# Jamol/kuma

Hardware: AMD Instinct MI355X
Metric: GiB/s device-resident WS frame mask/unmask, 64 KiB frames; % HBM peak (higher is better)
Workload: dtype u8

## Files before the change

### kuma_amd/csrc/kmws_utf8.hip

```cpp
#include "kmws_common.hpp"
#include "kmws_unmask_tile.hpp"
#include "kmws_utf8_dev.hpp"
#include "kmws_utf8_rule.hpp"

namespace kmws {

constexpr uint32_t kStatusBadStreams = kStatusBadDesc;

struct Utf8Ws {
    size_t plan_bytes;
    size_t first_bad, elems, aggs, pre, carry, total;
    uint32_t nblk;
};
static Utf8Ws utf8_ws_behind(size_t plan_bytes, uint32_t n, uint32_t n_streams)
{
    Utf8Ws w;
    w.nblk = (n + kBlock - 1) / kBlock;
    w.plan_bytes = plan_bytes;
    w.first_bad = r16(w.plan_bytes);
    w.elems = w.first_bad + r16((size_t)n * 4);
    w.aggs = w.elems + r16((size_t)n * 8);
    w.pre = w.aggs + r16((size_t)w.nblk * 8);
    w.carry = w.pre + r16((size_t)w.nblk * 8);
    w.total = w.carry + r16((size_t)n_streams * 8);
    return w;
}
static Utf8Ws utf8_ws(uint64_t span, uint32_t n, uint32_t n_streams)
{
    return utf8_ws_behind(kmws_unmask_workspace_size(span), n, n_streams);
}

__device__ __forceinline__ Utf8Elem block_scan(Utf8Elem e, Utf8Elem* s)
{
    const int tid = threadIdx.x;
    s[tid] = e;
    __syncthreads();
#pragma unroll
    for (int dlt = 1; dlt < kBlock; dlt <<= 1) {
        const Utf8Elem t = tid >= dlt ? utf8_combine(s[tid - dlt], s[tid]) : s[tid];
        __syncthreads();
        s[tid] = t;
        __syncthreads();
    }
    return s[tid];
}

__device__ __forceinline__ uint32_t stream_of(const uint32_t* __restrict__ first, uint32_t ns, uint32_t i)
{
    if (!first) return 0u;
    uint32_t lo = 0, hi = ns - 1;
    while (lo < hi) {
        const uint32_t mid = lo + (hi - lo + 1) / 2;
        if (first[mid] <= i) lo = mid; else hi = mid - 1;
    }
    return lo;
}
__device__ __forceinline__ uint32_t stream_begin(const uint32_t* __restrict__ first, uint32_t s)
{
    return first ? first[s] : 0u;
}
__device__ __forceinline__ uint32_t stream_end(const uint32_t* __restrict__ first, uint32_t n, uint32_t s)
{
    return first ? first[s + 1] : n;
}

__device__ __forceinline__ uint64_t load_carry(const kmws_utf8_carry* __restrict__ c, uint32_t s)
{
    uint64_t x = 0;
    if (c)
        for (int k = 0; k < 8; ++k) x |= (uint64_t)c[s].b[k] << (8 * k);
    return x;
}
__device__ __forceinline__ void store_carry(kmws_utf8_carry* __restrict__ c, uint32_t s, uint64_t x)
{
    for (int k = 0; k < 8; ++k) c[s].b[k] = (uint8_t)(x >> (8 * k));
}

__global__ void __launch_bounds__(kBlock) utf8_elem_kernel(const uint8_t* __restrict__ base, uint64_t span,
                                                           const kmws_desc* __restrict__ d,
                                                           const uint16_t* __restrict__ flags, uint32_t n, int masked,
                                                           const uint32_t* __restrict__ first, uint32_t ns,
                                                           const kmws_utf8_carry* __restrict__ carry_in,
                                                           Utf8Elem* __restrict__ elems, uint32_t* __restrict__ first_bad,
                                                           Utf8Elem* __restrict__ aggs, uint32_t nblk,
                                                           WsHead* __restrict__ head)
{
    __shared__ Utf8Elem s_scan[kBlock];
    const uint32_t i = blockIdx.x * kBlock + threadIdx.x;
    if (first && i <= ns) {
        const uint32_t x = first[i];
        if ((i == 0 && x != 0u) || (i == ns && x != n) || (i < ns && x > first[i + 1]))
            atomicOr(&head->status, kStatusBadStreams);
    }
    Utf8Elem e = utf8_identity();
    if (i < n) {
        const kmws_desc df = d[i];
        const uint32_t ob = flags[i] & 0xFFu, op = ob & 0x0Fu;
        uint32_t nb = 0, tail = 0;
        if (df.off > span || df.off + (uint64_t)df.len > span) {
            atomicOr(&head->status, kStatusBadDesc);
        } else if (op < 8u) {
            nb = df.len < 3u ? df.len : 3u;
            for (uint32_t k = 0; k < nb; ++k) {
                const uint32_t j = df.len - nb + k;
                uint32_t b = base[df.off + j];
                if (masked) b ^= (df.key >> (8u * (j & 3u))) & 0xFFu;
                tail = (tail << 8) | b;
            }
        }
        e = utf8_frame_elem(ob, i, tail, nb);
        uint32_t fb = kUtf8None;
        const uint32_t s = stream_of(first, ns, i);
        if (stream_begin(first, s) == i) {
            bool bad = false;
            const Utf8Elem st = utf8_carry_unpack(load_carry(carry_in, s), i, &bad);
            e = utf8_combine(st, e);
            if (bad && (op == 0u || op >= 8u)) fb = 0u;
        }
        elems[i] = e;
        first_bad[i] = fb;
    }
    const Utf8Elem inc = block_scan(e, s_scan);
    if (threadIdx.x == kBlock - 1 && blockIdx.x < nblk) aggs[blockIdx.x] = inc;
}

__global__ void __launch_bounds__(kBlock) utf8_scan_aggs_kernel(const Utf8Elem* __restrict__ aggs,
                                                                Utf8Elem* __restrict__ pre, uint32_t nblk)
{
    __shared__ Utf8Elem s_scan[kBlock];
    Utf8Elem run = utf8_identity();
    for (uint32_t c0 = 0; c0 < nblk; c0 += kBlock) {
        const uint32_t b = c0 + threadIdx.x;
        const Utf8Elem e = b < nblk ? aggs[b] : utf8_identity();
        block_scan(e, s_scan);
        const Utf8Elem ex = threadIdx.x ? s_scan[threadIdx.x - 1] : utf8_identity();
        if (b < nblk) pre[b] = utf8_combine(run, ex);
        run = utf8_combine(run, s_scan[kBlock - 1]);
        __syncthreads();
    }
}

__global__ void __launch_bounds__(kBlock) utf8_ctx_kernel(const uint16_t* __restrict__ flags, uint32_t n,
                                                          const uint32_t* __restrict__ first, uint32_t ns,
                                                          const kmws_utf8_carry* __restrict__ carry_in,
                                                          Utf8Elem* __restrict__ elems, const Utf8Elem* __restrict__ pre,
                                                          uint32_t* __restrict__ first_bad,
                                                          Utf8Elem* __restrict__ carry_tmp)
{
    __shared__ Utf8Elem s_scan[kBlock];
    const uint32_t i = blockIdx.x * kBlock + threadIdx.x;
    const Utf8Elem e = i < n ? elems[i] : utf8_identity();
    block_scan(e, s_scan);
    if (i >= n) return;
    Utf8Elem before = utf8_combine(pre[blockIdx.x], threadIdx.x ? s_scan[threadIdx.x - 1] : utf8_identity());
    const Utf8Elem after = utf8_combine(before, e);
    const uint32_t s = stream_of(first, ns, i);
    if (stream_begin(first, s) == i) {
        bool bad = false;
        before = utf8_carry_unpack(load_carry(carry_in, s), i, &bad);
    }
    const uint32_t ob = flags[i] & 0xFFu;
    const Utf8View v = utf8_frame_view(before, ob, i);
    elems[i] = Utf8Elem{v.slot, v.w};
    if ((v.w & kUtf8Checked) && (ob & 0x80u)) {
        const uint32_t nb = utf8_elem_nb(e);
        const uint32_t L = nb >= 3u ? utf8_elem_ctx(e) : (((v.w << (8u * nb)) | utf8_elem_ctx(e)) & 0xFFFFFFu);
        if (utf8_pending(L)) atomicMin(&first_bad[v.slot], i + 1u);
    }
    if (i + 1u == stream_end(first, n, s)) carry_tmp[s] = after;
}

constexpr int kUtf8V = (int)(kPlanTile / 16 / kBlock);
constexpr int kUtf8PolLoad = 2;
constexpr int kUtf8RsrcWord3 = 0x00020000;

__device__ __forceinline__ void covered_tile_check(const u32x4 (&v)[kUtf8V], const uint32_t (&prev)[kUtf8V],
                                                   uint32_t r, uint64_t lo, const kmws_desc& d0, Utf8View fv,
                                                   uint32_t f, uint32_t* __restrict__ first_bad)
{
    const int tid = threadIdx.x, lane = tid & 63;
    const uint64_t end = d0.off + d0.len;
    bool slow[kUtf8V];
    bool any = false;
#pragma unroll
    for (int i = 0; i < kUtf8V; ++i) {
        const uint64_t a = lo + 16u * (uint64_t)(tid + kBlock * i);
        const u32x4 w = v[i] ^ r;
        const uint32_t hb = (w.x | w.y | w.z | w.w) & 0x80808080u;
        slow[i] = hb != 0u || ((prev[i] ^ r) & 0x80000000u) != 0u || a < d0.off + 3u;
        any |= slow[i];
    }
    bool bad = false;
    if (__any(any)) {
#pragma unroll
        for (int i = 0; i < kUtf8V; ++i) {
            const uint64_t a = lo + 16u * (uint64_t)(tid + kBlock * i);
            if (slow[i]) bad |= word_bad(prev[i] ^ r, v[i] ^ r, a, d0.off, end, fv.w);
        }
    }
    const unsigned long long m = __ballot(bad);
    if (m != 0ull && lane == __ffsll((long long)m) - 1) report_bad(first_bad, fv.slot, f);
}

template <bool MASKED>
__device__ __forceinline__ void frames_check(const u32x4 (&v)[kUtf8V], const uint32_t (&prev)[kUtf8V], uint64_t lo,
                                             uint64_t hi, const kmws_desc* __restrict__ d, uint32_t f, uint32_t fl,
                                             const Utf8View* __restrict__ views, uint32_t* __restrict__ first_bad)
{
    const int tid = threadIdx.x;
#pragma unroll
    for (int i = 0; i < kUtf8V; ++i) {
        const uint64_t a = lo + 16u * (uint64_t)(tid + kBlock * i);
        if (a >= hi) continue;
        uint32_t gl = f, gh = fl + 1u;
        while (gl < gh) {
            const uint32_t mid = gl + (gh - gl) / 2;
            const kmws_desc dm = d[mid];
            if (dm.off + dm.len <= a) gl = mid + 1; else gh = mid;
        }
        for (uint32_t g = gl; g <= fl; ++g) {
            const kmws_desc dg = d[g];
            if (dg.off >= a + 16u) break;
            if (dg.len == 0u) continue;
            const Utf8View gv = views[g];
            if (!(gv.w & kUtf8Checked)) continue;
            const uint32_t r = MASKED ? rot_key(dg.key, dg.off) : 0u;
            if (plain_word_frame_bad(v[i] ^ r, prev[i] ^ r, a, dg.off, dg.off + dg.len, gv.w))
                report_bad(first_bad, gv.slot, g);
        }
    }
}

template <bool MASKED>
__global__ void __launch_bounds__(kBlock, MASKED ? 4 : 7) utf8_payload_kernel(const uint8_t* __restrict__ base, uint64_t span,
                                                              const kmws_desc* __restrict__ d, uint32_t n,
                                                              const TileRec* __restrict__ map,
                                                              const WsHead* __restrict__ head,
                                                              const Utf8View* __restrict__ views,
                                                              uint32_t* __restrict__ first_bad, TileMapping tm,
                                                              uint32_t b0)
{
    const int tid = threadIdx.x, lane = tid & 63, wave = tid >> 6;
    const uint32_t tile = tile_of_block(b0 + blockIdx.x, tm);
    const uint64_t lo = (uint64_t)tile * kPlanTile;
    const uint64_t hi = lo + kPlanTile < span ? lo + kPlanTile : span;
    const TileRecPair recs = *reinterpret_cast<const TileRecPair*>(map + tile);
    if (head->status != 0u) return;
    const bool cov = tile_rec_covered(recs.at, n);
    const uint32_t f = tile_rec_frame(recs.at, n);
    uint32_t fl = tile_rec_frame(recs.next, n);
    if (f >= n) return;
    if (fl >= n) fl = n - 1;
    if (fl < f) fl = f;

    Utf8View fv = Utf8View{0u, 0u};
    kmws_desc d0 = kmws_desc{0ull, 0u, 0u};
    if (cov) {
        fv = views[f];
        if (!(fv.w & kUtf8Checked)) return;
        d0 = d[f];
    } else {
        bool any = false;
        for (uint32_t g = f + (uint32_t)tid; g <= fl; g += kBlock) any |= (views[g].w & kUtf8Checked) != 0u;
        if (!__syncthreads_or(any)) return;
    }

    const __amdgpu_buffer_rsrc_t rs = __builtin_amdgcn_make_buffer_rsrc(
        const_cast<uint8_t*>(base) + lo, (short)0, (int)((hi - lo + 15) & ~15ull), kUtf8RsrcWord3);
    u32x4 v[kUtf8V];
#pragma unroll
    for (int i = 0; i < kUtf8V; ++i) {
        const uint32_t x = 16u * (uint32_t)(tid + kBlock * i);
        if (lo + x < hi) v[i] = __builtin_amdgcn_raw_buffer_load_b128(rs, (int)x, 0, kUtf8PolLoad);
        else v[i] = u32x4{0, 0, 0, 0};
    }
    uint32_t edge = 0;
    if (lane < kUtf8V) {
        const uint64_t ae = lo + 16u * (uint64_t)(64 * wave + kBlock * lane);
        if (ae >= 4u && ae <= span) edge = *reinterpret_cast<const uint32_t*>(base + ae - 4);
    }
    uint32_t prev[kUtf8V];
#pragma unroll
    for (int i = 0; i < kUtf8V; ++i) {
        const uint32_t up = __shfl_up(v[i].w, 1);
        const uint32_t ed = __shfl(edge, i);
        prev[i] = lane == 0 ? ed : up;
    }

    if (cov) {
        covered_tile_check(v, prev, MASKED ? recs.at.rkey : 0u, lo, d0, fv, f, first_bad);
        return;
    }

    frames_check<MASKED>(v, prev, lo, hi, d, f, fl, views, first_bad);
}

__global__ void __launch_bounds__(kBlock) utf8_finish_kernel(uint32_t n, const uint32_t* __restrict__ first,
                                                             uint32_t ns, const Utf8View* __restrict__ views,
                                                             const uint32_t* __restrict__ first_bad,
                                                             const Utf8Elem* __restrict__ carry_tmp,
                                                             const kmws_utf8_carry* __restrict__ carry_in,
                                                             kmws_utf8_carry* __restrict__ carry_out,
                                                             uint8_t* __restrict__ out)
{
    const uint32_t i = blockIdx.x * kBlock + threadIdx.x;
    if (i < n) {
        const Utf8View v = views[i];
        uint8_t r = KMWS_UTF8_NOT_TEXT;
        if (v.w & kUtf8Checked) {
            const uint32_t fb = first_bad[v.slot];
            r = fb > i + 1u ? KMWS_UTF8_OK : (fb == i + 1u ? KMWS_UTF8_BAD : KMWS_UTF8_AFTER_BAD);
        }
        out[i] = r;
    }
    if (carry_out && i < ns) {
        const uint32_t s = i;
        uint64_t c;
        if (stream_begin(first, s) >= stream_end(first, n, s)) {
            c = load_carry(carry_in, s);
        } else {
            const Utf8Elem after = carry_tmp[s];
            const bool chk = (after.w & (kUtf8Open | kUtf8Checked)) == (kUtf8Open | kUtf8Checked);
            c = utf8_carry_pack(after, chk && after.slot < n && first_bad[after.slot] != kUtf8None);
        }
        store_carry(carry_out, s, c);
    }
}

__global__ void __launch_bounds__(kBlock) utf8_carry_copy_kernel(uint32_t ns,
                                                                 const kmws_utf8_carry* __restrict__ carry_in,
                                                                 kmws_utf8_carry* __restrict__ carry_out)
{
    const uint32_t s = blockIdx.x * kBlock + threadIdx.x;
    if (s < ns) store_carry(carry_out, s, load_carry(carry_in, s));
}

constexpr int kFusedRows = (int)(kPlanTile / 1024);
constexpr uint32_t kFusedNoStore = 0x7FFFFFF0u;
static_assert(kUtf8V == kUnmaskV && kFusedRows == 4 * kUtf8V, "the validator's tile is the apply's");

constexpr unsigned kFusedBlocksPerCu = 4;
constexpr unsigned kFusedStaticLds = kUnmaskStaticLds + 4u * (unsigned)kFusedRows;

struct FusedWs {
    Utf8Ws u;
    size_t edges, total;
};
static FusedWs fused_ws(uint64_t span, uint32_t n, uint32_t n_streams)
{
    FusedWs w;
    w.u = utf8_ws(span, n, n_streams);
    const uint64_t ntiles = (span + kPlanTile - 1) / kPlanTile;
    w.edges = r16(w.u.total);
    w.total = w.edges + r16((size_t)ntiles * 4);
    return w;
}

__global__ void __launch_bounds__(kBlock) utf8_edges_kernel(const uint8_t* __restrict__ base,
                                                            uint32_t* __restrict__ edges, uint32_t ntiles)
{
    const uint32_t t = blockIdx.x * kBlock + threadIdx.x;
    if (t < ntiles) edges[t] = t ? *reinterpret_cast<const uint32_t*>(base + (uint64_t)t * kPlanTile - 4) : 0u;
}

__device__ __forceinline__ void fused_lookback(const u32x4 (&v)[kUtf8V], uint32_t edge, uint32_t* s_row,
                                               uint32_t (&prev)[kUtf8V])
{
    const int lane = threadIdx.x & 63, wave = threadIdx.x >> 6;
    if (lane == 63) {
#pragma unroll
        for (int i = 0; i < kUtf8V; ++i) s_row[wave + 4 * i] = v[i].w;
    }
    __syncthreads();
#pragma unroll
    for (int i = 0; i < kUtf8V; ++i) {
        const uint32_t up = __shfl_up(v[i].w, 1);
        const uint32_t ed = (wave == 0 && i == 0) ? edge : s_row[wave + 4 * i - 1];
        prev[i] = lane == 0 ? ed : up;
    }
}

__device__ __forceinline__ bool fused_word_frame_bad(const u32x4& v, uint32_t prev, uint64_t a, uint64_t off,
                                                     uint64_t end, uint32_t r, uint32_t ctx)
{
    return plain_word_frame_bad(v ^ r, prev ^ r, a, off, end, ctx);
}

template <bool FULL, bool TWO, bool NT>
__device__ __forceinline__ void fused_tile(uint8_t* __restrict__ base, uint64_t tile_lo, uint64_t tile_hi,
                                           const kmws_desc* __restrict__ d, uint32_t n, TileRec rec, TileRec rec_next,
                                           bool ok, const u32x4 (&v)[kUtf8V], uint32_t edge,
                                           const Utf8View* __restrict__ views, uint32_t* __restrict__ first_bad,
                                           uint64_t* s_off, uint64_t* s_end, uint32_t* s_key, uint32_t* s_row,
                                           const u32x4* pre)
{
    constexpr int V = kUtf8V;
    using Cfg = UnmaskCfg<V>;
    constexpr int SP = !NT ? kPolPlain : (TWO ? kPolStreamStoreLarge : kPolStreamStoreSmall);
    const int tid = threadIdx.x;
    const __amdgpu_buffer_rsrc_t rs = tile_rsrc(base, tile_lo, tile_hi);

    if (FULL && tile_rec_covered(rec, n)) {
        const uint32_t r = rec.rkey;
        const uint32_t f = tile_rec_frame(rec, n);
        const uint32_t fi = f < n ? f : 0u;
        const Utf8View fv = views[fi];
        const kmws_desc d0 = d[fi];
        const __amdgpu_buffer_rsrc_t rs_ok = __builtin_amdgcn_make_buffer_rsrc(
            base + tile_lo, (short)0, ok ? (int)Cfg::kTile : 0, kBufferRsrcWord3);
#pragma unroll
        for (int i = 0; i < V; ++i) {
            __builtin_amdgcn_sched_barrier(0);
            store_word<SP>(v[i] ^ r, rs_ok, 16u * (uint32_t)(tid + kBlock * i));
        }
        __builtin_amdgcn_sched_barrier(0);
        if (!ok | (f >= n) | !(fv.w & kUtf8Checked) | (d0.len == 0u) | (d0.off > tile_lo)) return;
        uint32_t prev[V];
        fused_lookback(v, edge, s_row, prev);
        covered_tile_check(v, prev, r, tile_lo, d0, fv, f, first_bad);
        return;
    }

    const uint32_t f0 = tile_rec_frame(rec, n);
    const uint32_t flast = tile_rec_frame(rec_next, n);
    const kmws_desc d0 = d[f0 < n ? f0 : 0];

    if (TWO && FULL && flast <= f0 + 1 && f0 < n) {
        const bool two = flast > f0 && flast < n;
        const kmws_desc d1 = two ? d[flast] : kmws_desc{~0ull, 0u, 0u};
        u32x4 m[V];
        const auto [r0, r1, s0, t0, s1, t1] = two_frame_masks(tile_lo, d0, d1, tid, m);
        const Utf8View v0 = views[f0];
        const Utf8View v1 = two ? views[flast] : Utf8View{0u, 0u};
        __builtin_amdgcn_sched_barrier(0);
#pragma unroll
        for (int i = 0; i < V; ++i) {
            const bool st = ok && (m[i].x | m[i].y | m[i].z | m[i].w) != 0u;
            store_word<SP>(v[i] ^ m[i], rs, st ? 16u * (uint32_t)(tid + kBlock * i) : kFusedNoStore);
        }
        if (!ok) return;
        const bool c0 = (v0.w & kUtf8Checked) != 0u && t0 > s0, c1 = (v1.w & kUtf8Checked) != 0u && t1 > s1;
        if (!c0 && !c1) return;
        uint32_t prev[V];
        fused_lookback(v, edge, s_row, prev);
#pragma unroll
        for (int i = 0; i < V; ++i) {
            const uint32_t x = 16u * (uint32_t)(tid + kBlock * i);
            const uint64_t a = tile_lo + x;
            if (c0 && s0 < x + 16 && t0 > x &&
                fused_word_frame_bad(v[i], prev[i], a, d0.off, d0.off + d0.len, r0, v0.w))
                report_bad(first_bad, v0.slot, f0);
            if (c1 && s1 < x + 16 && t1 > x &&
                fused_word_frame_bad(v[i], prev[i], a, d1.off, d1.off + d1.len, r1, v1.w))
                report_bad(first_bad, v1.slot, flast);
        }
        return;
    }

    u32x4 m[V];
    staged_masks(tile_lo, tile_hi, d, n, f0, flast, pre, s_off, s_end, s_key, tid, m);
    bool any = false;
    uint32_t fl = flast >= n ? n - 1 : flast;
    if (fl < f0) fl = f0;
    if (ok && f0 < n)
        for (uint32_t g = f0 + (uint32_t)tid; g <= fl; g += kBlock) any |= (views[g].w & kUtf8Checked) != 0u;
    if (__syncthreads_or(any)) {
        uint32_t prev[V];
        fused_lookback(v, edge, s_row, prev);
        frames_check<true>(v, prev, tile_lo, tile_hi, d, f0, fl, views, first_bad);
    }
#pragma unroll
    for (int i = 0; i < V; ++i) {
        const uint32_t x = 16u * (uint32_t)(tid + kBlock * i);
        const u32x4 mm = m[i];
        const bool st = ok && (mm.x | mm.y | mm.z | mm.w) != 0u;
        store_word<SP>(v[i] ^ mm, rs, st ? x : kFusedNoStore);
    }
}

template <bool TWO, bool NT>
__global__ void __launch_bounds__(kBlock) unmask_utf8_split_kernel(uint8_t* __restrict__ base,
                                                                   const kmws_desc* __restrict__ d, uint32_t n,
                                                                   const TileRec* __restrict__ map,
                                                                   const WsHead* __restrict__ head,
                                                                   const Utf8View* __restrict__ views,
                                                                   uint32_t* __restrict__ first_bad,
                                                                   const uint32_t* __restrict__ edges, TileMapping tm,
                                                                   uint32_t b0)
{
    using Cfg = UnmaskCfg<kUtf8V>;
    __shared__ uint64_t s_off[Cfg::kCap];
    __shared__ uint64_t s_end[Cfg::kCap];
    __shared__ uint32_t s_key[Cfg::kCap];
    __shared__ uint32_t s_row[kFusedRows];
    const uint32_t tile = tile_of_block(b0 + blockIdx.x, tm);
    const uint64_t lo = (uint64_t)tile * Cfg::kTile;
    const TileRecPair recs = *reinterpret_cast<const TileRecPair*>(map + tile);
    const TileRec rec = recs.at, rec_next = recs.next;
    const uint32_t status = head->status;
    const uint32_t edge = edges[tile];
    u32x4 v[kUtf8V];
    if constexpr (!TWO) {
        const uint32_t f = tile_rec_frame(rec, n), fl = tile_rec_frame(rec_next, n);
        const uint32_t fi = f + threadIdx.x;
        u32x4 pre = u32x4{0, 0, 0, 0};
        if (fi < n && fi <= fl) pre = *reinterpret_cast<const u32x4*>(d + fi);
        load_tile<kUtf8V, true>(base, lo, lo + Cfg::kTile, v);
        __builtin_amdgcn_sched_barrier(0);
        fused_tile<true, TWO, NT>(base, lo, lo + Cfg::kTile, d, n, rec, rec_next, (status & kStatusBadDesc) == 0, v,
                                  edge, views, first_bad, s_off, s_end, s_key, s_row, &pre);
        return;
    }
    __builtin_amdgcn_sched_barrier(0);
    load_tile<kUtf8V, true>(base, lo, lo + Cfg::kTile, v);
    __builtin_amdgcn_sched_barrier(0);
    fused_tile<true, TWO, NT>(base, lo, lo + Cfg::kTile, d, n, rec, rec_next, (status & kStatusBadDesc) == 0, v, edge,
                              views, first_bad, s_off, s_end, s_key, s_row, nullptr);
}

__global__ void __launch_bounds__(kBlock) unmask_utf8_tail_kernel(uint8_t* __restrict__ base, uint64_t span,
                                                                  const kmws_desc* __restrict__ d, uint32_t n,
                                                                  const TileRec* __restrict__ map,
                                                                  const WsHead* __restrict__ head,
                                                                  const Utf8View* __restrict__ views,
                                                                  uint32_t* __restrict__ first_bad,
                                                                  const uint32_t* __restrict__ edges, uint32_t tile)
{
    using Cfg = UnmaskCfg<kUtf8V>;
    __shared__ uint64_t s_off[Cfg::kCap];
    __shared__ uint64_t s_end[Cfg::kCap];
    __shared__ uint32_t s_key[Cfg::kCap];
    __shared__ uint32_t s_row[kFusedRows];
    const uint64_t tile_lo = (uint64_t)tile * Cfg::kTile;
    const uint32_t edge = edges[tile];
    u32x4 v[kUtf8V];
    load_tile<kUtf8V, false>(base, tile_lo, span, v);
    __builtin_amdgcn_sched_barrier(0);
    fused_tile<false, false, true>(base, tile_lo, span, d, n, map[tile], map[tile + 1],
                                   (head->status & kStatusBadDesc) == 0, v, edge, views, first_bad, s_off, s_end,
                                   s_key, s_row, nullptr);
}

static_assert(kPieceWords == kUtf8V * kBlock, "a piece is a tile of the validator: fused_lookback's rows");
__global__ void __launch_bounds__(kBlock) unmask_pieces_utf8_kernel(uint8_t* __restrict__ base,
                                                                    const kmws_desc* __restrict__ d,
                                                                    const Utf8View* __restrict__ views,
                                                                    const PieceRecEdge* __restrict__ pieces,
                                                                    uint8_t* __restrict__ verdict)
{
    constexpr int V = kUtf8V;
    __shared__ uint32_t s_row[kFusedRows];
    const PieceRecEdge pr = pieces[blockIdx.x];
    const kmws_desc x = d[pr.frame];
    const Utf8View fv = views[pr.frame];
    const PieceHull h = piece_hull(x, pr.piece);
    u32x4 v[V];
    load_piece(base, h, v);
    if (x.key != 0u) store_piece(base, x, h, v);
    if (!(fv.w & kUtf8Checked)) return;
    uint32_t prev[V];
    fused_lookback(v, pr.piece ? pr.edge : 0u, s_row, prev);
    bool bad = false;
#pragma unroll
    for (int i = 0; i < V; ++i) {
        const uint64_t w = h.w0 + threadIdx.x + (uint64_t)kBlock * i;
        if (w < h.w1) bad |= fused_word_frame_bad(v[i], prev[i], 16 * w, x.off, h.end, h.r, fv.w);
    }
    const unsigned long long m = __ballot(bad);
    if (m != 0ull && (int)(threadIdx.x & 63) == __ffsll((long long)m) - 1) verdict[fv.slot] = (uint8_t)1;
}

kmws_status launch_unmask_pieces_utf8(uint8_t* base, const kmws_desc* descs, const Utf8View* views,
                                      const PieceRecEdge* pieces, uint32_t np, uint8_t* verdict, hipStream_t s)
{
    if (np == 0) return KMWS_OK;
    if (!base || !descs || !views || !pieces || !verdict) return KMWS_ERR_INVALID_PARAM;
    hipLaunchKernelGGL(unmask_pieces_utf8_kernel, dim3(np), dim3(kBlock), 0, s, base, descs, views, pieces, verdict);
    return hip_status(hipGetLastError());
}

static bool have_device()
{
    static const bool have = kmws_device_count() > 0;
    return have;
}

kmws_status utf8_stream_args_check(bool ptrs_ok, const void* a, const void* b, uint32_t n, const uint32_t* stream_first,
                                   uint32_t n_streams, size_t need, size_t have)
{
    if (n >= 0x80000000u || n_streams >= 0x80000000u) return KMWS_ERR_INVALID_PARAM;
    if (n && !ptrs_ok) return KMWS_ERR_INVALID_PARAM;
    if ((reinterpret_cast<uintptr_t>(a) | reinterpret_cast<uintptr_t>(b)) & 15u) return KMWS_ERR_INVALID_PARAM;
    if (n && (n_streams == 0u || (!stream_first && n_streams != 1u))) return KMWS_ERR_INVALID_PARAM;
    if (have < need) return KMWS_ERR_BUFFER_TOO_SMALL;
    if (!have_device()) return KMWS_ERR_NOT_SUPPORTED;
    return KMWS_OK;
}

struct Utf8Arrays {
    WsHead* head;
    const TileRec* map;
    uint32_t* first_bad;
    Utf8Elem *elems, *aggs, *pre, *carry_tmp;
    const Utf8View* views;
};
static Utf8Arrays utf8_arrays(void* workspace, const Utf8Ws& w)
{
    uint8_t* wsb = static_cast<uint8_t*>(workspace);
    Utf8Arrays a;
    a.head = static_cast<WsHead*>(workspace);
    a.map = reinterpret_cast<const TileRec*>(a.head + 1);
    a.first_bad = reinterpret_cast<uint32_t*>(wsb + w.first_bad);
    a.elems = reinterpret_cast<Utf8Elem*>(wsb + w.elems);
    a.aggs = reinterpret_cast<Utf8Elem*>(wsb + w.aggs);
    a.pre = reinterpret_cast<Utf8Elem*>(wsb + w.pre);
    a.carry_tmp = reinterpret_cast<Utf8Elem*>(wsb + w.carry);
    a.views = reinterpret_cast<const Utf8View*>(a.elems);
    return a;
}
static void launch_utf8_frames(const Utf8Ws& w, const Utf8Arrays& a, const uint8_t* base, uint64_t span,
                               const kmws_desc* descs, const uint16_t* flags, uint32_t n, int masked,
                               const uint32_t* stream_first, uint32_t n_streams, const kmws_utf8_carry* carry_in,
                               hipStream_t s)
{
    const uint32_t sblk = stream_first ? (n_streams + 1u + kBlock - 1) / kBlock : 0u;
    hipLaunchKernelGGL(utf8_elem_kernel, dim3(w.nblk > sblk ? w.nblk : sblk), dim3(kBlock), 0, s, base, span, descs,
                       flags, n, masked, stream_first, n_streams, carry_in, a.elems, a.first_bad, a.aggs, w.nblk,
                       a.head);
    hipLaunchKernelGGL(utf8_scan_aggs_kernel, dim3(1), dim3(kBlock), 0, s, a.aggs, a.pre, w.nblk);
    hipLaunchKernelGGL(utf8_ctx_kernel, dim3(w.nblk), dim3(kBlock), 0, s, flags, n, stream_first, n_streams, carry_in,
                       a.elems, a.pre, a.first_bad, a.carry_tmp);
}
static void launch_utf8_finish(const Utf8Arrays& a, uint32_t n, const uint32_t* stream_first, uint32_t n_streams,
                               const kmws_utf8_carry* carry_in, kmws_utf8_carry* carry_out, uint8_t* out, hipStream_t s)
{
    const uint32_t fin_lanes = carry_out && n_streams > n ? n_streams : n;
    hipLaunchKernelGGL(utf8_finish_kernel, dim3((fin_lanes + kBlock - 1) / kBlock), dim3(kBlock), 0, s, n,
                       stream_first, n_streams, a.views, a.first_bad, a.carry_tmp, carry_in, carry_out, out);
}
static kmws_status launch_carry_copy(uint32_t n_streams, const kmws_utf8_carry* carry_in, kmws_utf8_carry* carry_out,
                                     hipStream_t s)
{
    if (carry_out && n_streams)
        hipLaunchKernelGGL(utf8_carry_copy_kernel, dim3((n_streams + kBlock - 1) / kBlock), dim3(kBlock), 0, s,
                           n_streams, carry_in, carry_out);
    return hip_status(hipGetLastError());
}

size_t utf8_frame_arrays_size(uint32_t n, uint32_t n_streams) { return utf8_ws_behind(0, n, n_streams).total; }

static Utf8Arrays frame_arrays(void* arrays, WsHead* head, const Utf8Ws& w)
{
    Utf8Arrays a = utf8_arrays(arrays, w);
    a.head = head;
    a.map = nullptr;
    return a;
}
Utf8FrameArrays launch_utf8_frame_state(void* arrays, WsHead* head, const uint8_t* base, uint64_t span,
                                        const kmws_desc* descs, const uint16_t* flags, uint32_t n, int masked,
                                        const uint32_t* stream_first, uint32_t n_streams,
                                        const kmws_utf8_carry* carry_in, hipStream_t s)
{
    const Utf8Ws w = utf8_ws_behind(0, n, n_streams);
    const Utf8Arrays a = frame_arrays(arrays, head, w);
    launch_utf8_frames(w, a, base, span, descs, flags, n, masked, stream_first, n_streams, carry_in, s);
    return Utf8FrameArrays{a.views, a.first_bad};
}
void launch_utf8_frame_finish(void* arrays, uint32_t n, const uint32_t* stream_first, uint32_t n_streams,
                              const kmws_utf8_carry* carry_in, kmws_utf8_carry* carry_out, uint8_t* out,
                              hipStream_t s)
{
    const Utf8Arrays a = frame_arrays(arrays, nullptr, utf8_ws_behind(0, n, n_streams));
    launch_utf8_finish(a, n, stream_first, n_streams, carry_in, carry_out, out, s);
}
kmws_status launch_utf8_carry_copy(uint32_t n_streams, const kmws_utf8_carry* carry_in, kmws_utf8_carry* carry_out,
                                   hipStream_t s)
{
    return launch_carry_copy(n_streams, carry_in, carry_out, s);
}

static kmws_status fused_check(const uint8_t* base, bool ptrs_ok, uint32_t n, const uint32_t* stream_first,
                               uint32_t n_streams, uint64_t span, int schedule, size_t workspace_bytes,
                               const FusedWs& w, uint32_t* code)
{
    *code = schedule < 0 ? default_schedule(span, n) : (uint32_t)schedule;
    if (!valid_schedule(*code)) return KMWS_ERR_INVALID_PARAM;
    return utf8_stream_args_check(ptrs_ok, base, nullptr, n, stream_first, n_streams, n ? w.total : 0, workspace_bytes);
}

static kmws_status launch_fused(uint32_t code, uint8_t* base, uint64_t span, const kmws_desc* descs,
                                const uint16_t* flags, uint32_t n, const uint32_t* stream_first, uint32_t n_streams,
                                const kmws_utf8_carry* carry_in, kmws_utf8_carry* carry_out, uint8_t* out,
                                void* workspace, const FusedWs& w, hipStream_t s)
{
    Split sp;
    if (!split_of(code & 0xFFu, &sp)) return KMWS_ERR_INVALID_PARAM;
    const Utf8Arrays a = utf8_arrays(workspace, w.u);
    uint32_t* edges = reinterpret_cast<uint32_t*>(static_cast<uint8_t*>(workspace) + w.edges);
    const uint64_t ntiles = (span + kPlanTile - 1) / kPlanTile;
    const uint64_t nfull = span / kPlanTile;
    if (ntiles)
        hipLaunchKernelGGL(utf8_edges_kernel, dim3((uint32_t)((ntiles + kBlock - 1) / kBlock)), dim3(kBlock), 0, s,
                           base, edges, (uint32_t)ntiles);
    launch_utf8_frames(w.u, a, base, span, descs, flags, n, 1, stream_first, n_streams, carry_in, s);

    const unsigned lds_pad = unmask_capped(span, n) ? lds_pad_for(kFusedBlocksPerCu, kFusedStaticLds) : 0u;
    const TileMapping tm = tile_mapping((uint32_t)nfull, sp);
    launch_split_grid(nfull, lds_pad, temporal_stores(code), [&](auto two, auto nt, dim3 grid, uint32_t b0, unsigned pad) {
        hipLaunchKernelGGL((unmask_utf8_split_kernel<decltype(two)::value, decltype(nt)::value>), grid, dim3(kBlock), pad,
                           s, base, descs, n, a.map, a.head, a.views, a.first_bad, edges, tm, b0);
    });
    if (ntiles > nfull)
        hipLaunchKernelGGL(unmask_utf8_tail_kernel, dim3(1), dim3(kBlock), 0, s, base, span, descs, n, a.map, a.head,
                           a.views, a.first_bad, edges, (uint32_t)nfull);
    launch_utf8_finish(a, n, stream_first, n_streams, carry_in, carry_out, out, s);
    return hip_status(hipGetLastError());
}

}

using namespace kmws;

extern "C" {

size_t kmws_utf8_workspace_size(uint64_t span, uint32_t n, uint32_t n_streams)
{
    return utf8_ws(span, n, n_streams).total;
}

kmws_status kmws_utf8_validate(const uint8_t* base, uint64_t span, const kmws_desc* descs, const uint16_t* flags,
                               uint32_t n, int payload_masked, const uint32_t* stream_first, uint32_t n_streams,
                               const kmws_utf8_carry* carry_in, kmws_utf8_carry* carry_out, uint8_t* out,
                               void* workspace, size_t workspace_bytes, void* stream)
{
    const Utf8Ws w = utf8_ws(span, n, n_streams);
    kmws_status st = utf8_stream_args_check(base && descs && flags && out && workspace, base, nullptr, n, stream_first,
                                            n_streams, n ? w.total : 0, workspace_bytes);
    if (st != KMWS_OK) return st;
    hipStream_t s = static_cast<hipStream_t>(stream);
    if (n == 0) return launch_carry_copy(n_streams, carry_in, carry_out, s);
    st = launch_plan(span, descs, n, workspace, w.plan_bytes, s);
    if (st != KMWS_OK) return st;
    note_device_batch(span, s);

    const Utf8Arrays a = utf8_arrays(workspace, w);
    WsHead* head = a.head;
    const TileRec* map = a.map;
    uint32_t* first_bad = a.first_bad;
    const Utf8View* views = a.views;
    const int masked = payload_masked != 0;
    launch_utf8_frames(w, a, base, span, descs, flags, n, masked, stream_first, n_streams, carry_in, s);

    const uint64_t ntiles = (span + kPlanTile - 1) / kPlanTile;
    Split sp;
    (void)split_of(KMWS_SCHED_SPLIT4, &sp);
    const TileMapping tm = tile_mapping((uint32_t)(span / kPlanTile), sp);
    launch_split_grid(ntiles, 0u, false, [&](auto, auto, dim3 grid, uint32_t b0, unsigned) {
        if (masked)
            hipLaunchKernelGGL(utf8_payload_kernel<true>, grid, dim3(kBlock), 0, s, base, span, descs, n, map, head,
                               views, first_bad, tm, b0);
        else
            hipLaunchKernelGGL(utf8_payload_kernel<false>, grid, dim3(kBlock), 0, s, base, span, descs, n, map, head,
                               views, first_bad, tm, b0);
    });
    launch_utf8_finish(a, n, stream_first, n_streams, carry_in, carry_out, out, s);
    return hip_status(hipGetLastError());
}

size_t kmws_unmask_utf8_workspace_size(uint64_t span, uint32_t n, uint32_t n_streams)
{
    return fused_ws(span, n, n_streams).total;
}

kmws_status kmws_unmask_utf8_batch(uint8_t* base, uint64_t span, const kmws_desc* descs, const uint16_t* flags,
                                   uint32_t n, const uint32_t* stream_first, uint32_t n_streams,
                                   const kmws_utf8_carry* carry_in, kmws_utf8_carry* carry_out, uint8_t* out,
                                   void* workspace, size_t workspace_bytes, int schedule, void* stream)
{
    const FusedWs w = fused_ws(span, n, n_streams);
    uint32_t code = 0;
    kmws_status st = fused_check(base, base && descs && flags && out && workspace, n, stream_first, n_streams, span,
                                 schedule, workspace_bytes, w, &code);
    if (st != KMWS_OK) return st;
    hipStream_t s = static_cast<hipStream_t>(stream);
    if (n == 0) return launch_carry_copy(n_streams, carry_in, carry_out, s);
    st = launch_plan(span, descs, n, workspace, w.u.plan_bytes, s);
    if (st != KMWS_OK) return st;
    note_device_batch(2 * span, s);
    return launch_fused(code, base, span, descs, flags, n, stream_first, n_streams, carry_in, carry_out, out, workspace,
                        w, s);
}

kmws_status kmws_unpack_unmask_utf8(uint8_t* wire, uint64_t wire_len, const uint64_t* hdr_off, uint32_t n, int mode,
                                    kmws_desc* out_desc, uint16_t* out_flags, uint8_t* out_err,
                                    const uint32_t* stream_first, uint32_t n_streams, const kmws_utf8_carry* carry_in,
                                    kmws_utf8_carry* carry_out, uint8_t* out_utf8, void* workspace,
                                    size_t workspace_bytes, int schedule, void* stream)
{
    const FusedWs w = fused_ws(wire_len, n, n_streams);
    uint32_t code = 0;
    if (mode != KMWS_MODE_CLIENT && mode != KMWS_MODE_SERVER) return KMWS_ERR_INVALID_PARAM;
    const bool fits = (wire_len + kPlanTile - 1) / kPlanTile <= 0x7FFFFFFFull;
    kmws_status st = fused_check(wire, wire && hdr_off && out_desc && out_flags && out_utf8 && workspace && fits, n,
                                 stream_first, n_streams, wire_len, schedule, workspace_bytes, w, &code);
    if (st != KMWS_OK) return st;
    hipStream_t s = static_cast<hipStream_t>(stream);
    if (n == 0) return launch_carry_copy(n_streams, carry_in, carry_out, s);
    st = launch_unpack_plan(wire, wire_len, hdr_off, n, mode, out_desc, out_flags, out_err, workspace, s);
    if (st != KMWS_OK) return st;
    note_device_batch(2 * wire_len, s);
    return launch_fused(code, wire, wire_len, out_desc, out_flags, n, stream_first, n_streams, carry_in, carry_out,
                        out_utf8, workspace, w, s);
}

}
```

### kuma_amd/csrc/kmws_utf8_dev.hpp

```cpp
#pragma once
#include "kmws_common.hpp"
#include "kmws_utf8_rule.hpp"

namespace kmws {

constexpr uint32_t kUtf8None = 0xFFFFFFFFu;

__device__ __forceinline__ uint32_t window_byte(uint32_t prev, const u32x4& w, int r)
{
    const uint32_t dw = r < 0 ? prev : (r < 4 ? w.x : (r < 8 ? w.y : (r < 12 ? w.z : w.w)));
    return (dw >> (8u * ((uint32_t)r & 3u))) & 0xFFu;
}

__device__ __forceinline__ bool word_bad(uint32_t prev, const u32x4& w, uint64_t a, uint64_t off, uint64_t end,
                                         uint32_t ctx)
{
    const bool deep = off + 3u <= a;
    if (deep && end >= a + 16u) return utf8_word_bad_swar(prev, w.x, w.y, w.z, w.w);
    const int s = deep ? -3 : (int)((int64_t)off - (int64_t)a);
    const int e = end >= a + 16u ? 16 : (int)(end - a);
    uint32_t L = deep ? 0u : (ctx & 0xFFFFFFu);
    bool bad = false;
#pragma unroll 1
    for (int r = s; r < e; ++r) {
        const uint32_t b = window_byte(prev, w, r);
        if (r >= 0) bad |= utf8_byte_bad(b, L);
        L = utf8_append(L, b);
    }
    return bad;
}

__device__ __forceinline__ bool plain_word_frame_bad(const u32x4& w, uint32_t prev, uint64_t a, uint64_t off,
                                                     uint64_t end, uint32_t ctx)
{
    const bool plain = off + 3u <= a && end >= a + 16u && ((w.x | w.y | w.z | w.w) & 0x80808080u) == 0u &&
                       (prev & 0x80000000u) == 0u;
    return !plain && word_bad(prev, w, a, off, end, ctx);
}

__device__ __forceinline__ void report_bad(uint32_t* __restrict__ first_bad, uint32_t slot, uint32_t frame)
{
    if (__builtin_nontemporal_load(&first_bad[slot]) > frame + 1u) atomicMin(&first_bad[slot], frame + 1u);
}

struct Utf8FrameArrays {
    const Utf8View* views;
    uint32_t* first_bad;
};
size_t utf8_frame_arrays_size(uint32_t n, uint32_t n_streams);
Utf8FrameArrays launch_utf8_frame_state(void* arrays, WsHead* head, const uint8_t* base, uint64_t span,
                                        const kmws_desc* descs, const uint16_t* flags, uint32_t n, int masked,
                                        const uint32_t* stream_first, uint32_t n_streams,
                                        const kmws_utf8_carry* carry_in, hipStream_t s);
void launch_utf8_frame_finish(void* arrays, uint32_t n, const uint32_t* stream_first, uint32_t n_streams,
                              const kmws_utf8_carry* carry_in, kmws_utf8_carry* carry_out, uint8_t* out,
                              hipStream_t s);
kmws_status launch_utf8_carry_copy(uint32_t n_streams, const kmws_utf8_carry* carry_in, kmws_utf8_carry* carry_out,
                                   hipStream_t s);
kmws_status utf8_stream_args_check(bool ptrs_ok, const void* a, const void* b, uint32_t n, const uint32_t* stream_first,
                                   uint32_t n_streams, size_t need, size_t have);

}
```

### kuma_amd/csrc/kmws_utf8_rule.hpp

```cpp
#pragma once
#ifdef __HIPCC__
#include <hip/hip_runtime.h>
#endif
#include <stdint.h>

#ifndef __host__
#define __host__
#endif
#ifndef __device__
#define __device__
#endif
#define KMWS_HD __host__ __device__ inline

namespace kmws {

KMWS_HD uint32_t utf8_append(uint32_t L, uint32_t b) { return ((L << 8) | (b & 0xFFu)) & 0xFFFFFFu; }

KMWS_HD uint32_t utf8_need3(uint32_t p1, uint32_t p2, uint32_t p3)
{
    const uint32_t lead = (p1 - 0xC2u) <= 0x32u;
    const uint32_t cont1 = (p1 & 0xC0u) == 0x80u;
    const uint32_t second = (p2 - 0xE0u) <= 0x14u;
    const uint32_t third = (uint32_t)((p2 & 0xC0u) == 0x80u) & (uint32_t)((p3 - 0xF0u) <= 4u);
    const uint32_t need = lead | (cont1 & (second | third));
    const uint32_t lo = p1 == 0xE0u ? 0xA0u : (p1 == 0xF0u ? 0x90u : 0x80u);
    const uint32_t hi = p1 == 0xEDu ? 0x9Fu : (p1 == 0xF4u ? 0x8Fu : 0xBFu);
    return need ? (lo | (hi << 8)) : 0u;
}
KMWS_HD uint32_t utf8_need(uint32_t L) { return utf8_need3(L & 0xFFu, (L >> 8) & 0xFFu, (L >> 16) & 0xFFu); }

KMWS_HD bool utf8_byte_bad3(uint32_t b, uint32_t p1, uint32_t p2, uint32_t p3)
{
    const uint32_t need = utf8_need3(p1, p2, p3);
    const uint32_t lo = need & 0xFFu, hi = need >> 8;
    const uint32_t bad_cont = (b - lo) > (hi - lo);
    const uint32_t bad_start = (uint32_t)(b >= 0x80u) & (uint32_t)((b - 0xC2u) > 0x32u);
    return (need ? bad_cont : bad_start) != 0u;
}
KMWS_HD bool utf8_byte_bad(uint32_t b, uint32_t L)
{
    return utf8_byte_bad3(b, L & 0xFFu, (L >> 8) & 0xFFu, (L >> 16) & 0xFFu);
}

struct Utf8Swar {
    uint32_t cont, lead234, lead34, lead4, e0, ed, f0, f4, bad, ge_a0, ge_90;
};
KMWS_HD Utf8Swar utf8_swar_classes(uint32_t x)
{
    const uint32_t hi = x & 0x80808080u, t = (x & 0x7F7F7F7Fu) | 0x80808080u;
#define KMWS_GE(K) (hi & (t - ((uint32_t)(K) - 0x80u) * 0x01010101u))
    const uint32_t c0 = KMWS_GE(0xC0), c2 = KMWS_GE(0xC2), e0 = KMWS_GE(0xE0), e1 = KMWS_GE(0xE1);
    const uint32_t ed = KMWS_GE(0xED), ee = KMWS_GE(0xEE), f0 = KMWS_GE(0xF0), f1 = KMWS_GE(0xF1);
    const uint32_t f4 = KMWS_GE(0xF4), f5 = KMWS_GE(0xF5);
    Utf8Swar c;
    c.ge_a0 = KMWS_GE(0xA0);
    c.ge_90 = KMWS_GE(0x90);
#undef KMWS_GE
    c.cont = hi & ~c0;
    c.lead234 = c2 & ~f5;
    c.lead34 = e0 & ~f5;
    c.lead4 = f0 & ~f5;
    c.e0 = e0 & ~e1;
    c.ed = ed & ~ee;
    c.f0 = f0 & ~f1;
    c.f4 = f4 & ~f5;
    c.bad = (c0 & ~c2) | f5;
    return c;
}
KMWS_HD uint32_t utf8_swar_back(uint32_t cur, uint32_t before, uint32_t nb)
{
    return (cur << (8u * nb)) | (before >> (32u - 8u * nb));
}
KMWS_HD uint32_t utf8_swar_dword(const Utf8Swar& c, const Utf8Swar& p)
{
    const uint32_t due = utf8_swar_back(c.lead234, p.lead234, 1) | utf8_swar_back(c.lead34, p.lead34, 2) |
                         utf8_swar_back(c.lead4, p.lead4, 3);
    return (due ^ c.cont) | c.bad | (utf8_swar_back(c.e0, p.e0, 1) & ~c.ge_a0) |
           (utf8_swar_back(c.ed, p.ed, 1) & c.ge_a0) | (utf8_swar_back(c.f0, p.f0, 1) & ~c.ge_90) |
           (utf8_swar_back(c.f4, p.f4, 1) & c.ge_90);
}
KMWS_HD bool utf8_word_bad_swar(uint32_t prev, uint32_t x0, uint32_t x1, uint32_t x2, uint32_t x3)
{
    const Utf8Swar cp = utf8_swar_classes(prev), c0 = utf8_swar_classes(x0), c1 = utf8_swar_classes(x1),
                   c2 = utf8_swar_classes(x2), c3 = utf8_swar_classes(x3);
    const uint32_t err = utf8_swar_dword(c0, cp) | utf8_swar_dword(c1, c0) | utf8_swar_dword(c2, c1) |
                         utf8_swar_dword(c3, c2);
    return (err & 0x80808080u) != 0u;
}

KMWS_HD bool utf8_pending(uint32_t L) { return utf8_need(L) != 0u; }

struct Utf8Elem {
    uint32_t slot;
    uint32_t w;
};
constexpr uint32_t kUtf8Open = 1u << 26, kUtf8Checked = 1u << 27, kUtf8Reset = 1u << 28;
KMWS_HD uint32_t utf8_elem_ctx(Utf8Elem e) { return e.w & 0xFFFFFFu; }
KMWS_HD uint32_t utf8_elem_nb(Utf8Elem e) { return (e.w >> 24) & 3u; }
KMWS_HD Utf8Elem utf8_identity() { return Utf8Elem{0u, 0u}; }

KMWS_HD Utf8Elem utf8_combine(Utf8Elem a, Utf8Elem b)
{
    if (b.w & kUtf8Reset) return b;
    const uint32_t nb = utf8_elem_nb(b), na = utf8_elem_nb(a);
    const uint32_t ctx = nb >= 3u ? utf8_elem_ctx(b) : (((utf8_elem_ctx(a) << (8u * nb)) | utf8_elem_ctx(b)) & 0xFFFFFFu);
    const uint32_t n = na + nb > 3u ? 3u : na + nb;
    return Utf8Elem{a.slot, ctx | (n << 24) | (a.w & (kUtf8Open | kUtf8Checked | kUtf8Reset))};
}

KMWS_HD Utf8Elem utf8_frame_elem(uint32_t op_byte, uint32_t i, uint32_t tail, uint32_t nb)
{
    const uint32_t op = op_byte & 0x0Fu, fin = op_byte & 0x80u, rsv1 = op_byte & 0x40u;
    const uint32_t bytes = (tail & 0xFFFFFFu) | (nb << 24);
    if (op >= 8u) return utf8_identity();
    if (fin) return Utf8Elem{i, bytes | kUtf8Reset};
    if (op == 0u) return Utf8Elem{0u, bytes};
    return Utf8Elem{i, bytes | kUtf8Reset | kUtf8Open | ((op == 1u && !rsv1) ? kUtf8Checked : 0u)};
}

struct Utf8View {
    uint32_t slot;
    uint32_t w;
};
KMWS_HD Utf8View utf8_frame_view(Utf8Elem before, uint32_t op_byte, uint32_t i)
{
    const uint32_t op = op_byte & 0x0Fu, rsv1 = op_byte & 0x40u;
    if (op >= 8u) return Utf8View{i, 0u};
    if (op != 0u) return Utf8View{i, (op == 1u && !rsv1) ? kUtf8Checked : 0u};
    if ((before.w & (kUtf8Open | kUtf8Checked)) != (kUtf8Open | kUtf8Checked)) return Utf8View{i, 0u};
    return Utf8View{before.slot, utf8_elem_ctx(before) | kUtf8Checked};
}

constexpr uint32_t kUtf8CarryOpen = 1u, kUtf8CarryChecked = 2u, kUtf8CarryBad = 4u;
KMWS_HD uint64_t utf8_carry_pack(Utf8Elem after, bool bad)
{
    if (!(after.w & kUtf8Open)) return 0ull;
    if (!(after.w & kUtf8Checked)) return (uint64_t)kUtf8CarryOpen;
    return (uint64_t)(kUtf8CarryOpen | kUtf8CarryChecked | (bad ? kUtf8CarryBad : 0u)) |
           ((uint64_t)utf8_elem_ctx(after) << 8);
}
KMWS_HD Utf8Elem utf8_carry_unpack(uint64_t c, uint32_t slot, bool* bad)
{
    const uint32_t f = (uint32_t)c & 0xFFu;
    *bad = (f & kUtf8CarryOpen) && (f & kUtf8CarryChecked) && (f & kUtf8CarryBad);
    if (!(f & kUtf8CarryOpen)) return Utf8Elem{slot, kUtf8Reset};
    if (!(f & kUtf8CarryChecked)) return Utf8Elem{slot, kUtf8Reset | kUtf8Open};
    return Utf8Elem{slot, ((uint32_t)(c >> 8) & 0xFFFFFFu) | (3u << 24) | kUtf8Reset | kUtf8Open | kUtf8Checked};
}

}
```

Baseline: 3157.

## Replace SWAR UTF-8 validator with perm-based nibble lookup tables

The full-word UTF-8 check now uses a three-nibble lookup-table scheme built on v_perm_b32 and alignbyte, replacing the class-mask SWAR evaluation. The aim is fewer ALU instructions per 16-byte word in the payload kernel. Launch bounds for both masked and unmasked kernels change to 8 waves per EU, which limits registers and may cause spills. The new tables and the final-byte check must reproduce the old validator exactly, which is a correctness risk.

```diff
diff --git a/kuma_amd/csrc/kmws_utf8.hip b/kuma_amd/csrc/kmws_utf8.hip
--- a/kuma_amd/csrc/kmws_utf8.hip
+++ b/kuma_amd/csrc/kmws_utf8.hip
@@ -232,7 +232,7 @@
 }
 
 template <bool MASKED>
-__global__ void __launch_bounds__(kBlock, MASKED ? 4 : 7) utf8_payload_kernel(const uint8_t* __restrict__ base, uint64_t span,
+__global__ void __launch_bounds__(kBlock, 8) utf8_payload_kernel(const uint8_t* __restrict__ base, uint64_t span,
                                                               const kmws_desc* __restrict__ d, uint32_t n,
                                                               const TileRec* __restrict__ map,
                                                               const WsHead* __restrict__ head,
diff --git a/kuma_amd/csrc/kmws_utf8_dev.hpp b/kuma_amd/csrc/kmws_utf8_dev.hpp
--- a/kuma_amd/csrc/kmws_utf8_dev.hpp
+++ b/kuma_amd/csrc/kmws_utf8_dev.hpp
@@ -16,7 +16,7 @@
                                          uint32_t ctx)
 {
     const bool deep = off + 3u <= a;
-    if (deep && end >= a + 16u) return utf8_word_bad_swar(prev, w.x, w.y, w.z, w.w);
+    if (deep && end >= a + 16u) return utf8_word_bad_lut(prev, w.x, w.y, w.z, w.w);
     const int s = deep ? -3 : (int)((int64_t)off - (int64_t)a);
     const int e = end >= a + 16u ? 16 : (int)(end - a);
     uint32_t L = deep ? 0u : (ctx & 0xFFFFFFu);
diff --git a/kuma_amd/csrc/kmws_utf8_rule.hpp b/kuma_amd/csrc/kmws_utf8_rule.hpp
--- a/kuma_amd/csrc/kmws_utf8_rule.hpp
+++ b/kuma_amd/csrc/kmws_utf8_rule.hpp
@@ -88,6 +88,82 @@
     return (err & 0x80808080u) != 0u;
 }
 
+constexpr uint32_t kU8Short = 0x01, kU8Long = 0x02, kU8Over3 = 0x04, kU8Large = 0x08, kU8Surr = 0x10, kU8Over2 = 0x20,
+                   kU8Large80 = 0x40, kU8Over4 = 0x40, kU8TwoConts = 0x80;
+constexpr uint32_t kU8Carry = kU8Short | kU8Long | kU8TwoConts;
+constexpr uint32_t utf8_tab4(uint32_t e0, uint32_t e1, uint32_t e2, uint32_t e3)
+{
+    return e0 | (e1 << 8) | (e2 << 16) | (e3 << 24);
+}
+constexpr uint32_t kU8T1Ascii = kU8Long * 0x01010101u;
+constexpr uint32_t kU8T1_8 = kU8TwoConts * 0x01010101u;
+constexpr uint32_t kU8T1_C = utf8_tab4(kU8Short | kU8Over2, kU8Short, kU8Short | kU8Over3 | kU8Surr,
+                                       kU8Short | kU8Large | kU8Large80 | kU8Over4);
+constexpr uint32_t kU8T2_0 = utf8_tab4(kU8Carry | kU8Over3 | kU8Over2 | kU8Over4, kU8Carry | kU8Over2, kU8Carry, kU8Carry);
+constexpr uint32_t kU8T2_4 = utf8_tab4(kU8Carry | kU8Large, kU8Carry | kU8Large | kU8Large80,
+                                       kU8Carry | kU8Large | kU8Large80, kU8Carry | kU8Large | kU8Large80);
+constexpr uint32_t kU8T2_8 = (kU8Carry | kU8Large | kU8Large80) * 0x01010101u;
+constexpr uint32_t kU8T2_C = kU8T2_8 | (kU8Surr << 8);
+constexpr uint32_t kU8T3Ascii = kU8Short * 0x01010101u;
+constexpr uint32_t kU8T3_8 =
+    utf8_tab4(kU8Long | kU8Over2 | kU8TwoConts | kU8Over3 | kU8Large80 | kU8Over4,
+              kU8Long | kU8Over2 | kU8TwoConts | kU8Over3 | kU8Large, kU8Long | kU8Over2 | kU8TwoConts | kU8Surr | kU8Large,
+              kU8Long | kU8Over2 | kU8TwoConts | kU8Surr | kU8Large);
+constexpr uint32_t kU8T3_C = kU8Short * 0x01010101u;
+
+KMWS_HD uint32_t utf8_alignbyte(uint32_t hi, uint32_t lo, uint32_t n)
+{
+#if defined(__HIP_DEVICE_COMPILE__)
+    return __builtin_amdgcn_alignbyte(hi, lo, n);
+#else
+    return (uint32_t)((((uint64_t)hi << 32) | lo) >> (8u * (n & 3u)));
+#endif
+}
+KMWS_HD uint32_t utf8_perm(uint32_t hi, uint32_t lo, uint32_t sel)
+{
+#if defined(__HIP_DEVICE_COMPILE__)
+    return __builtin_amdgcn_perm(hi, lo, sel);
+#else
+    const uint64_t in = ((uint64_t)hi << 32) | lo;
+    uint8_t pick[16];
+    for (uint32_t s = 0; s < 8u; ++s) pick[s] = (uint8_t)(in >> (8u * s));
+    for (uint32_t s = 8; s < 12u; ++s) pick[s] = ((in >> (16u * (s - 8u) + 15u)) & 1u) ? 0xFFu : 0u;
+    pick[12] = 0u;
+    pick[13] = pick[14] = pick[15] = 0xFFu;
+    uint32_t r = 0;
+    for (uint32_t k = 0; k < 4u; ++k) {
+        const uint32_t s = (sel >> (8u * k)) & 0xFFu;
+        r |= (uint32_t)pick[s < 15u ? s : 15u] << (8u * k);
+    }
+    return r;
+#endif
+}
+KMWS_HD uint32_t utf8_sign_bytes(uint32_t x) { return utf8_perm(x << 8, x, 0x090B080Au); }
+KMWS_HD uint32_t utf8_lut_ge(uint32_t x, uint32_t k)
+{
+    return x & 0x80808080u & ((x & 0x7F7F7F7Fu) + (0x100u - k) * 0x01010101u);
+}
+KMWS_HD uint32_t utf8_lut_dword(uint32_t x, uint32_t before)
+{
+    const uint32_t p1 = utf8_alignbyte(x, before, 3);
+    const uint32_t m1 = utf8_sign_bytes(p1), m3 = utf8_sign_bytes(x);
+    const uint32_t h1 = utf8_perm(kU8T1_C, kU8T1_8, (p1 >> 4) & 0x07070707u);
+    const uint32_t h3 = utf8_perm(kU8T3_C, kU8T3_8, (x >> 4) & 0x07070707u);
+    const uint32_t t1 = (h1 & m1) | (kU8T1Ascii & ~m1);
+    const uint32_t t3 = (h3 & m3) | (kU8T3Ascii & ~m3);
+    const uint32_t s2 = p1 & 0x07070707u, m2 = utf8_sign_bytes(p1 << 4);
+    const uint32_t l2 = utf8_perm(kU8T2_4, kU8T2_0, s2), u2 = utf8_perm(kU8T2_C, kU8T2_8, s2);
+    const uint32_t t2 = (u2 & m2) | (l2 & ~m2);
+    const uint32_t due23 = utf8_lut_ge(utf8_alignbyte(x, before, 2), 0xE0u) | utf8_lut_ge(utf8_alignbyte(x, before, 1), 0xF0u);
+    return (t1 & t2 & t3) ^ due23;
+}
+KMWS_HD bool utf8_word_bad_lut(uint32_t prev, uint32_t x0, uint32_t x1, uint32_t x2, uint32_t x3)
+{
+    const uint32_t err = utf8_lut_dword(x0, prev) | utf8_lut_dword(x1, x0) | utf8_lut_dword(x2, x1) | utf8_lut_dword(x3, x2);
+    const bool last = (x3 - 0xC0000000u) < 0x02000000u || x3 >= 0xF5000000u;
+    return err != 0u || last;
+}
+
 KMWS_HD bool utf8_pending(uint32_t L) { return utf8_need(L) != 0u; }
 
 struct Utf8Elem {
```

Result: no change. 3149 (-0.3%).
